# cvg/diffmvs

Measured on AMD Instinct MI355X. Metric: depth-maps/sec (640x512, 5 src views), higher is better.
Workload: dtype f32

## Files before the change

### diffmvs_amd/_lib.py

```python
from __future__ import annotations

import ctypes as C
import os

PKG = os.path.dirname(os.path.abspath(__file__))
HIP_LIB_PATH = os.environ.get("DMVS_LIB") or os.path.join(PKG, "libdmvs_hip.so")

ACT_NONE, ACT_RELU, ACT_SIGMOID, ACT_TANH, ACT_SILU = range(5)
IN_PLAIN, IN_UPSAMPLE2, IN_UNSHUFFLE2, IN_ZEROINSERT2 = range(4)
LAYOUT_NCHW, LAYOUT_NHWC, LAYOUT_NHWC_BF16, LAYOUT_NHWC_F16 = 0, 1, 2, 3
DTYPE_F32, DTYPE_BF16, DTYPE_F16, DTYPE_F32_PLAIN = 0, 1, 2, 3
ARITH_F32, ARITH_BF16, ARITH_SPLIT = 0, 1, 2
EW_DEPTH_TO_DISP, EW_DISP_TO_DEPTH = 0, 1

_P = C.c_void_p
_I = C.c_int32
_F = C.c_float


class Conv2dDesc(C.Structure):
    _fields_ = [
        ("in0", _P), ("in1", _P), ("mul0", _P), ("weight", _P), ("scale", _P), ("shift", _P),
        ("residual", _P), ("gru_z", _P), ("gru_h", _P), ("out", _P), ("gn_stats", _P), ("out_mul", _P),
        ("B", _I), ("c0", _I), ("c1", _I), ("Hin", _I), ("Win", _I), ("Hout", _I), ("Wout", _I),
# ... 13 lines not shown
    ]


class GetCostDesc(C.Structure):
    _fields_ = [
        ("ref", _P), ("src", _P), ("rt", _P), ("inv_depth", _P), ("confidence", _P), ("view_w", _P),
        ("disp_min", _P), ("disp_max", _P), ("out_cost", _P), ("out_samples", _P), ("worklist", _P),
        ("B", _I), ("S", _I), ("C", _I), ("G", _I), ("n", _I), ("H", _I), ("W", _I), ("vw_shift", _I),
        ("cost_cstride", _I), ("cost_coffset", _I), ("samp_cstride", _I), ("samp_coffset", _I),
        ("interval", _F), ("min_radius", _F), ("max_radius", _F), ("feat_dtype", _I), ("tune", _I),
    ]


SIGNATURES = {
    "dmvs_abi_version": [],
    "dmvs_conv2d_f32": [C.POINTER(Conv2dDesc), _P],
    "dmvs_featurenet_stem_f32": [_P, _P, _P, _P, _P, _P, _P, _P, _I, _I, _I, _I, _P],
    "dmvs_featurenet_stem3_f32": [_P, _P, _P, _P, _P, _P, _P, _P, _P, _P, _P, _I, _I, _I, _I, _P],
    "dmvs_featurenet_conv1_pair_f32": [_P, _P, _P, _P, _P, _P, _P, _P, _I, _I, _I, _I, _P],
    "dmvs_featurenet_fpn_tail_f32": [_P, _P, _P, _P, _P, _P, _I, _I, _I, _I, _P],
    "dmvs_conv2d_wgrad_workspace_f32": [C.POINTER(Conv2dDesc), C.POINTER(C.c_int64)],
    "dmvs_conv2d_wgrad_f32": [C.POINTER(Conv2dDesc), _P, _P, _P, _P, C.c_int64, _P],
    "dmvs_conv3d_f32": [C.POINTER(Conv3dDesc), _P],
    "dmvs_conv3d_wgrad_workspace_f32": [C.POINTER(Conv3dDesc), C.POINTER(C.c_int64)],
    "dmvs_conv3d_wgrad_f32": [C.POINTER(Conv3dDesc), _P, _P, _P, _P, C.c_int64, _P],
    "dmvs_compose_proj_f32": [_P, _P, _I, _I, _P],
    "dmvs_warp_volume_f32": [_P, _P, _P, _P, _I, _I, _I, _I, _I, _I, _I, _P],
    "dmvs_getcost_quad_f32": [C.POINTER(GetCostDesc), _P],
    "dmvs_warp_corr_init_quad_f32": [_P, _P, _P, _P, _P, _P, _I, _I, _I, _I, _I, _I, _I, _I, _I, _I, _I, _P],
    "dmvs_warp_corr_init_bwd_f32": [_P, _P, _P, _P, _P, _P, _P, _P, _I, _I, _I, _I, _I, _I, _I, _I, _I, _I, _P],
    "dmvs_getcost_bwd_f32": [C.POINTER(GetCostDesc), _P, _P, _P, _P],
    "dmvs_view_aggregate_bwd_f32": [_P, _P, _P, _P, _P, _P, _I, _I, _I, _I, _P],
    "dmvs_view_aggregate_f32": [_P, _P, _P, _I, _I, _I, _I, _P],
    "dmvs_sigmoid_max_d_f32": [_P, _P, _I, _I, _I, _P],
    "dmvs_depth_regress_f32": [_P, _P, _P, _P, _P, _P, _I, _I, _I, _P],
    "dmvs_convex_upsample_f32": [_P, _P, _P, _P, _P, _P, _I, _I, _I, _I, _P],
    "dmvs_mask_upsample4_f32": [_P, _P, _P, _F, _P, _P, _P, _P, _P, _I, _I, _I, _I, _I, _P],
    "dmvs_groupnorm_silu_f32": [_P, _P, _P, _P, _P, _P, _P, _I, _I, _I, _I, _F, _P],
    "dmvs_groupnorm_apply_f32": [_P, _P, _P, _P, _P, _P, _P, _I, _I, _I, _I, _F, _P],
    "dmvs_delta_update_f32": [_P, _P, _P, _F, _P, _P, _P, _I, _I, _I, _I, _P],
    "dmvs_depth_convert_f32": [_P, _P, _P, _P, _I, _I, _I, _P],
    "dmvs_act_slice_f32": [_P, _P, _I, _I, _I, _I, _I, _I, _I, _I, _P],
    "dmvs_upsample_nearest_f32": [_P, _P, _I, _I, _I, _I, _P],
    "dmvs_nchw_to_nhwc_f32": [_P, _P, _I, _I, _I, _P],
    "dmvs_groupnorm_silu_bwd_workspace_f32": [_I, _I, _I, C.POINTER(C.c_int64)],
    "dmvs_groupnorm_silu_bwd_f32": [_P, _P, _P, _P, _P, _P, _P, _P, _P, _P, _P, C.c_int64, _I, _I, _I, _I, _F, _P],
    "dmvs_batchnorm_workspace_f32": [_I, _I, _I, _I, C.POINTER(C.c_int64)],
    "dmvs_batchnorm_train_fwd_f32": [_P, _P, _P, _P, _P, _P, _P, _P, _P, C.c_int64, _I, _I, _I, _I, _I, _F, _F, _I, _P],
    "dmvs_batchnorm_train_bwd_f32": [_P, _P, _P, _P, _P, _P, _P, _P, _P, _P, C.c_int64, _I, _I, _I, _I, _I, _I, _P],
    "dmvs_geo_consistency_f32": [_P, _P, _P, _P, _P, _I, _I, _F, _F, _P, _P, _I, _I, _I, _I, _I, _P],
    "dmvs_sumsq_f32": [_P, C.c_int64, _P, _P],
    "dmvs_adamw_step_f32": [_P, _P, _P, _P, C.c_int64, _F, _F, _F, _F, _F, _I, _F, _P, _F, _P],
    "dmvs_view_select_scores_f64": [_P, _P, _P, _P, _P, C.c_int64, C.c_int64, _P, _I, C.c_double, C.c_double, C.c_double, _P, _P, _P],
    "dmvs_cloud_nn_dist_f32": [_P, C.c_int64, _P, C.c_int64, _P, _P, C.c_int64, _P, C.c_double, _P, _F, _P, _P, _P],
    "dmvs_cloud_stats_f32": [_P, _P, C.c_int64, _F, _P, _I, C.c_double, _I, _P, _P],
    "dmvs_cloud_nn_index_f32": [_P, C.c_int64, _P, C.c_int64, _P, _P, C.c_int64, _P, C.c_double, _P, _F, _P, _P, _P, _P, _P],
    "dmvs_cloud_pair_moments_f64": [_P, C.c_int64, _P, _P, C.c_int64, _P, _P, _F, _P, _P, C.c_double, C.c_double, C.c_double, _I, _P, _P],
    "dmvs_cloud_crop_prism_f32": [_P, C.c_int64, _P, _P, _I, _I, C.c_double, C.c_double, _P, _P],
    "dmvs_depth_stats_f32": [_P, _P, _P, C.c_int64, C.c_int64, _P, _I, C.c_double, C.c_double, C.c_double, C.c_double, _I, _P, _P],
    "dmvs_cloud_splat_zmin_f32": [_P, C.c_int64, _P, _P, C.c_int64, _I, _I, C.c_double, C.c_double, C.c_double, _I, _I, _P, _P, _P, _P],
    "dmvs_cloud_splat_sum_f32": [_P, C.c_int64, _P, _P, C.c_int64, _I, _I, C.c_double, C.c_double, C.c_double, C.c_double, C.c_double, _I, _P, _P, _P, _P],
    "dmvs_depth_normals_f32": [_P, _P, _P, C.c_int64, _I, _I, _I, C.c_double, _I, _P, _P, _P],
    "dmvs_tsdf_integrate_f32": [_P, _P, _P, _P, C.c_int64, _I, _I, _I, _I, _I, _P, C.c_double, C.c_double, _I, _P, _P, _P, _P],
    "dmvs_tsdf_flags_u8": [_P, _P, _I, _I, _I, _I, _P, _P, _P],
    "dmvs_tsdf_vertices_f32": [_P, _P, _P, _I, _I, _I, _P, C.c_double, _P, _P, C.c_int64, _P, _P, _P],
    "dmvs_tsdf_faces_i32": [_P, _I, _I, _I, _P, _P, _P, C.c_int64, _P, _P],
    "dmvs_mesh_raster_fill_u64": [_P, C.c_int64, _P],
    "dmvs_mesh_raster_zid_u64": [_P, C.c_int64, _P, C.c_int64, _P, _P, C.c_int64, _I, _I, _I, _I, _P, _P, _P, _P, C.c_int64, _P],
    "dmvs_mesh_raster_resolve_f32": [_P, _P, C.c_int64, _P, C.c_int64, _P, _P, C.c_int64, _I, _I, _P, _P, _P, _P, _P, _P],
    "dmvs_mesh_label_round_i32": [_P, C.c_int64, C.c_int64, _P, _P, _I, _P],
    "dmvs_mesh_face_tally_i64": [_P, C.c_int64, _P, C.c_int64, _P, C.c_double, C.c_double, _P, _P, _P, _I, _P],
    "dmvs_mesh_sample_f32": [_P, C.c_int64, _P, C.c_int64, _P, C.c_int64, C.c_int64, _P, _P, _I, _P],
}
VIEW_SELECT_MAX_IMAGES, VIEW_SELECT_MAX_LIST = 16384, 1 << 23
CLOUD_MAX_RINGS, CLOUD_MAX_KEY_BITS, CLOUD_MAX_THRESHOLDS = 1024, 62, 16
CLOUD_MOMENTS, CLOUD_MAX_POLYGON = 20, 256
DEPTH_MAX_THRESHOLDS, DEPTH_SLOTS = 8, 7
SPLAT_VIEW_CHUNK, SPLAT_VIEW_DOUBLES, SPLAT_SLOTS, SPLAT_MAX_RADIUS, SPLAT_NO_PRETEST = 8, 15, 4, 16, 0x1
NORMAL_MAX_RADIUS, NORMAL_CAM_DOUBLES, NORMAL_VIEW_CHUNK, NORMAL_SLOTS = 4, 27, 8, 4
TSDF_VIEW_CHUNK, TSDF_VIEW_DOUBLES, TSDF_MAX_VIEWS, TSDF_MAX_QUADS, TSDF_NO_CULL = 8, 12, 65535, 357913941, 0x1
RASTER_VIEW_DOUBLES, RASTER_SLOTS, RASTER_SMALL, RASTER_CULL_NEG, RASTER_CULL_POS = 22, 8, 64, 0x1, 0x2
ABI_VERSION = 4
TUNE_NO_WALK, TUNE_PIECES4, TUNE_NO_LEAN, TUNE_1X1_TILED, TUNE_NO_TALL, TUNE_TALL = 0x4, 0x8, 0x100, 0x200, 0x400, 0x800
TUNE3D_PIECES4, TUNE3D_S2_DIRECT, TUNE3D_NO_PAIR = 0x1, 0x2, 0x4
TUNE_SWEEP_GLOBAL = 0x1
TUNE_WGRAD_ACCUMULATE = 0x1000
TUNE_SPLIT_ALL = 0x20000
TUNE_STEM_EXACT = 0x40000


def tune_xcd_group(n: int) -> int:
    return (int(n) & 7) << 14


def tune3d_xcd_group(n: int) -> int:
    return (int(n) & 7) << 4
TUNE_BWD_INTERLEAVED, BWD_GATHER_INTERLEAVED = 0x1, 2


def tune_tile_wx(n: int) -> int:
    return n & 3


def tune_tile_mt(n: int) -> int:
    return (n & 7) << 4


class DmvsError(RuntimeError):
    pass


class Lib:

    def __init__(self, path: str):
        if not os.path.exists(path):
            raise DmvsError(f"{path} not found: build it with `python -m diffmvs_amd.build`")
        self.path = path
        self.dll = C.CDLL(path)
        self.dll.dmvs_abi_version.restype = C.c_int
        v = self.dll.dmvs_abi_version()
        if v != ABI_VERSION:
            raise DmvsError(f"{path}: ABI version {v}, binding expects {ABI_VERSION} (rebuild: python -m diffmvs_amd.build)")
        for name, argtypes in SIGNATURES.items():
            fn = getattr(self.dll, name)
            fn.argtypes = argtypes
            fn.restype = C.c_int

    def call(self, name: str, *args):
        rc = getattr(self.dll, name)(*args)
        if rc != 0:
            raise DmvsError(f"{name} failed with code {rc}" + (" (DMVS_EINVAL: unsupported descriptor)" if rc == -22 else " (hipError_t)"))


_hip_lib = None


def hip_lib() -> Lib:
    global _hip_lib
    if _hip_lib is None:
        _hip_lib = Lib(HIP_LIB_PATH)
    return _hip_lib
```

### diffmvs_amd/csrc/conv3d.hip

```cpp

#include <type_traits>

#include "dmvs_common.h"
#include "dmvs_lds_poison.h"

typedef float f32x4 __attribute__((ext_vector_type(4)));
typedef float f32x2 __attribute__((ext_vector_type(2)));

__device__ __forceinline__ int conv3d_xcd_tile(int tile, int ntiles, int tune) {
    const int xg = (tune >> 4) & 7;
    if (xg == 1) return tile;
    const unsigned g = xg == 0 ? 4u : (xg <= 4 ? 1u << (xg - 1) : 4u);
    return (int)dmvs_xcd_grouped_block((unsigned)tile, (unsigned)ntiles, g);
}

constexpr int pad16mod32_3d(int n) {
    int m = n;
    while (m % 32 != 16) ++m;
    return m;
}

constexpr unsigned kHaloGuard = 0x00808080u;

template <int ID, int IH, int IW, int PLANE_>
// ... 667 lines not shown
                __builtin_amdgcn_global_load_lds(srcp, DMVS_LDS_PTR(dstp), 16, 0, 0);
            }
        }
    };

    const int xr = tid / XT, lx = (tid - xr * XT) * 4;
    const int rd = xr / YT, ry = xr - rd * YT;
    const bool active = rd < DT;
    const int lbase = 4 + ((2 * rd) * IH + 2 * ry) * PW + lx;
    float acc[2][2][4];
#pragma unroll
    for (int i = 0; i < 16; ++i) (&acc[0][0][0])[i] = 0.0f;
    stage(0, lds);
    int cur = 0;
    for (int ci = 0; ci < d.cin; ++ci, cur ^= 1) {
        const float* s_in = lds + cur * plane + lbase;
        DMVS_DMA_BARRIER();
        if (ci + 1 < d.cin) stage(ci + 1, lds + (cur ^ 1) * plane);
        if (!active) continue;
        typedef const __attribute__((address_space(4))) float* cfloat_p;
        cfloat_p wc = (cfloat_p)(uintptr_t)(d.weight + ci * 27 * d.cout_pad);
        float w[27];
#pragma unroll
        for (int t = 0; t < 27; ++t) w[t] = wc[t * d.cout_pad];
#pragma unroll
        for (int dz = 0; dz < 4; ++dz) {
#pragma unroll
            for (int yy = 0; yy < 4; ++yy) {
                const float* row = s_in + (dz * IH + yy) * PW;
                const f32x4 mid = *reinterpret_cast<const f32x4*>(row);
                const float in6[6] = {row[-1], mid[0], mid[1], mid[2], mid[3], row[4]};
#pragma unroll
                for (int od = 0; od < 2; ++od) {
#pragma unroll
                    for (int oy = 0; oy < 2; ++oy) {
                        const int kd = dz - od, ky = yy - oy;
                        if (kd < 0 || kd > 2 || ky < 0 || ky > 2) continue;
                        const float w0 = w[(kd * 3 + ky) * 3], w1 = w[(kd * 3 + ky) * 3 + 1], w2 = w[(kd * 3 + ky) * 3 + 2];
#pragma unroll
                        for (int j = 0; j < 4; ++j)
                            acc[od][oy][j] = fmaf(in6[j], w0, fmaf(in6[j + 1], w1, fmaf(in6[j + 2], w2, acc[od][oy][j])));
                    }
                }
            }
        }
    }
    if (!active) return;
    const int ovol = d.Dout * d.Hout * d.Wout;
    const float sc = d.scale ? d.scale[0] : 1.0f, sh = d.shift ? d.shift[0] : 0.0f;
    float* outb = d.out + (size_t)b * ovol;
    const float* resb = d.residual ? d.residual + (size_t)b * ovol : nullptr;
#pragma unroll
    for (int od = 0; od < 2; ++od) {
#pragma unroll
        for (int oy = 0; oy < 2; ++oy) {
            const int gd = d0 + 2 * rd + od, gy = y0 + 2 * ry + oy;
            if (gd >= d.Dout || gy >= d.Hout) continue;
            const int o0 = (gd * d.Hout + gy) * d.Wout + lx;
            f32x4 y;
#pragma unroll
            for (int j = 0; j < 4; ++j) y[j] = dmvs_act(acc[od][oy][j] * sc + sh, d.act);
            if (resb) y += *reinterpret_cast<const f32x4*>(resb + o0);
            *reinterpret_cast<f32x4*>(outb + o0) = y;
        }
    }
}

static bool c1_rows_shape(const dmvs_conv3d_desc& d, int& XT, int& YT, int& DT) {
    if (d.Win % 4 || d.Win < 16 || d.Win > 256) return false;
    if (((uintptr_t)d.in | (uintptr_t)d.out | (uintptr_t)d.residual) & 15) return false;
    XT = d.Win / 4;
    const int RT = DMVS_BLOCK / XT;
    long best_tiles = -1, best_rows = 0;
    for (int yt = 1; yt <= 4 && yt <= RT; ++yt)
        for (int dt = 1; dt <= 4 && yt * dt <= RT; ++dt) {
            const long rows = (long)(2 * yt + 2) * (2 * dt + 2);
            if (2 * (rows * (d.Win + 4) + 4) > kC1RowsLds || rows * (XT + 1) + 1 > kC1RowsPieces * DMVS_BLOCK) continue;
            const long tiles = (long)((d.Hout + 2 * yt - 1) / (2 * yt)) * ((d.Dout + 2 * dt - 1) / (2 * dt));
            if (best_tiles < 0 || tiles < best_tiles || (tiles == best_tiles && tiles * rows < best_rows)) {
                best_tiles = tiles; best_rows = tiles * rows; YT = yt; DT = dt;
            }
        }
    return best_tiles > 0;
}


template <int CO>
__device__ __forceinline__ void conv3d_epilogue(const dmvs_conv3d_desc& d, const float (&acc)[CO], int co0, int b,
                                                size_t ovox) {
    const size_t ovol = (size_t)d.Dout * d.Hout * d.Wout;
#pragma unroll
    for (int co = 0; co < CO; ++co) {
        const int cg = co0 + co;
        if (cg >= d.cout) break;
        float y = acc[co];
        if (d.scale) y *= d.scale[cg];
        if (d.shift) y += d.shift[cg];
        y = dmvs_act(y, d.act);
        const size_t oi = ((size_t)b * d.cout + cg) * ovol + ovox;
        if (d.residual) y += d.residual[oi];
        d.out[oi] = y;
    }
}

template <int CO, int STRIDE>
__global__ void __launch_bounds__(DMVS_BLOCK) conv3d_kernel(const dmvs_conv3d_desc d) {
    const long total = (long)d.B * d.Dout * d.Hout * d.Wout;
    const long p = (long)blockIdx.x * DMVS_BLOCK + threadIdx.x;
    const int co0 = blockIdx.y * CO;
    const bool live = p < total;
    long q = live ? p : total - 1;
    const int ox = (int)(q % d.Wout); q /= d.Wout;
    const int oy = (int)(q % d.Hout); q /= d.Hout;
    const int od = (int)(q % d.Dout);
    const int b = (int)(q / d.Dout);

    float acc[CO];
#pragma unroll
    for (int i = 0; i < CO; ++i) acc[i] = 0.0f;
    const size_t ivol = (size_t)d.Din * d.Hin * d.Win;
    const int id0 = od * STRIDE - 1, iy0 = oy * STRIDE - 1, ix0 = ox * STRIDE - 1;
    for (int ci = 0; ci < d.cin; ++ci) {
        const float* vol = d.in + ((size_t)b * d.cin + ci) * ivol;
        const float* wrow = d.weight + (size_t)ci * 27 * d.cout_pad + co0;
#pragma unroll
        for (int kd = 0; kd < 3; ++kd) {
            const int id = id0 + kd;
            const bool din = id >= 0 && id < d.Din;
#pragma unroll
            for (int ky = 0; ky < 3; ++ky) {
                const int iy = iy0 + ky;
                const bool yin = din && iy >= 0 && iy < d.Hin;
#pragma unroll
                for (int kx = 0; kx < 3; ++kx) {
                    const int ix = ix0 + kx;
                    float v = 0.0f;
                    if (yin && ix >= 0 && ix < d.Win) v = vol[((size_t)id * d.Hin + iy) * d.Win + ix];
                    const float* wt = wrow + ((kd * 3 + ky) * 3 + kx) * d.cout_pad;
#pragma unroll
                    for (int co = 0; co < CO; ++co) acc[co] = fmaf(v, wt[co], acc[co]);
                }
            }
        }
    }
    if (!live) return;
    conv3d_epilogue<CO>(d, acc, co0, b, ((size_t)od * d.Hout + oy) * d.Wout + ox);
}

template <int CO>
__global__ void __launch_bounds__(DMVS_BLOCK) deconv3d_kernel(const dmvs_conv3d_desc d) {
    const long total = (long)d.B * d.Din * d.Hin * d.Win;
    const long p = (long)blockIdx.x * DMVS_BLOCK + threadIdx.x;
    const int co0 = blockIdx.y * CO;
    const int pd = (blockIdx.z >> 2) & 1, py = (blockIdx.z >> 1) & 1, px = blockIdx.z & 1;
    const bool live = p < total;
    long q = live ? p : total - 1;
    const int jx = (int)(q % d.Win); q /= d.Win;
    const int jy = (int)(q % d.Hin); q /= d.Hin;
    const int jd = (int)(q % d.Din);
    const int b = (int)(q / d.Din);

    float acc[CO];
#pragma unroll
    for (int i = 0; i < CO; ++i) acc[i] = 0.0f;
    const size_t ivol = (size_t)d.Din * d.Hin * d.Win;
    const int nd = pd ? 2 : 1, ny = py ? 2 : 1, nx = px ? 2 : 1;
// ... 107 lines not shown
    const int jx = jx0 + m, jd = jd0 + wave;
    const bool live = jx < d.Win && jd < d.Din;
    float* outb = d.out + (size_t)b * d.cout * ovol;
    const float* resb = d.residual ? d.residual + (size_t)b * d.cout * ovol : nullptr;
#pragma unroll
    for (int r = 0; r < 4; ++r) {
        const int cg = cg0 + r;
        const bool okc = cg < d.cout;
        const float sc = d.scale ? d.scale[okc ? cg : 0] : 1.0f, sh = d.shift ? d.shift[okc ? cg : 0] : 0.0f;
#pragma unroll
        for (int c2 = 0; c2 < 2; ++c2) {
#pragma unroll
            for (int mt = 0; mt < 4; ++mt) {
                const float keep = lowhalf ? acc[c2][mt][r] : acc[c2 + 2][mt][r];
                const float give = lowhalf ? acc[c2 + 2][mt][r] : acc[c2][mt][r];
                const float got = __shfl_xor(give, 32, 64);
                const int c = lowhalf ? c2 : c2 + 2;
                const int jy = jy0 + mt;
                if (!live || !okc || jy >= d.Hin) continue;
                const int o = cg * ovol + ((2 * jd + (c >> 1)) * d.Hout + 2 * jy + (c & 1)) * d.Wout + 2 * jx;
                float v0 = dmvs_act((lowhalf ? keep : got) * sc + sh, d.act);
                float v1 = dmvs_act((lowhalf ? got : keep) * sc + sh, d.act);
                if (resb) {
                    const float2 rv = *reinterpret_cast<const float2*>(resb + o);
                    v0 += rv.x;
                    v1 += rv.y;
                }
                *reinterpret_cast<float2*>(outb + o) = make_float2(v0, v1);
            }
        }
    }
}

static bool conv3d_s2_mfma(const dmvs_conv3d_desc& d) { return !(d.tune & DMVS_TUNE3D_S2_DIRECT); }

extern "C" int dmvs_conv3d_f32(const dmvs_conv3d_desc* dp, void* stream) {
    if (!dp) return DMVS_EINVAL;
    const dmvs_conv3d_desc& d = *dp;
    hipStream_t st = (hipStream_t)stream;
    if (d.cout_pad % 8 || d.cout > d.cout_pad || !d.in || !d.weight || !d.out) return DMVS_EINVAL;
    if ((uintptr_t)d.weight & 15) return DMVS_EINVAL;
    const int co = (d.cout_pad % 16 == 0) ? 16 : 8;
    dim3 block(DMVS_BLOCK);
    if (d.transposed) {
        if (d.stride != 2 || d.Dout != 2 * d.Din || d.Hout != 2 * d.Hin || d.Wout != 2 * d.Win) return DMVS_EINVAL;
        const long total = (long)d.B * d.Din * d.Hin * d.Win;
        if ((long)d.cout * d.Dout * d.Hout * d.Wout < (1L << 31) && (long)d.cin * d.Din * d.Hin * d.Win < (1L << 31)) {
            const int tiles_x = (d.Win + 15) / 16, tiles_y = (d.Hin + 3) / 4, tiles_d = (d.Din + 3) / 4;
            dim3 g((unsigned)(tiles_x * tiles_y * tiles_d * d.B), (unsigned)((d.cout + 7) / 8));
            hipLaunchKernelGGL(deconv3d_mfma_kernel, g, block, 0, st, d, tiles_x, tiles_y, tiles_d);
            return dmvs_launch_status();
        }
        dim3 grid(dmvs_ceil_div(total, DMVS_BLOCK), d.cout_pad / co, 8);
        if (co == 16) hipLaunchKernelGGL((deconv3d_kernel<16>), grid, block, 0, st, d);
        else hipLaunchKernelGGL((deconv3d_kernel<8>), grid, block, 0, st, d);
        return dmvs_launch_status();
    }
    if (d.stride != 1 && d.stride != 2) return DMVS_EINVAL;
    const int ed = (d.Din - 1) / d.stride + 1, eh = (d.Hin - 1) / d.stride + 1, ew = (d.Win - 1) / d.stride + 1;
    if (ed != d.Dout || eh != d.Hout || ew != d.Wout) return DMVS_EINVAL;
    const long total = (long)d.B * d.Dout * d.Hout * d.Wout;
    dim3 grid(dmvs_ceil_div(total, DMVS_BLOCK), d.cout_pad / co);
    if (d.stride == 1 && ((long)d.cin * d.Din * d.Hin * d.Win >= (1L << 31) || (long)d.cout * d.Dout * d.Hout * d.Wout >= (1L << 31)))
        return DMVS_EINVAL;
    if (d.stride == 1 && d.cout == 1) {
        int XT, YT, DT;
        if (c1_rows_shape(d, XT, YT, DT)) {
            const int tiles_y = (d.Hout + 2 * YT - 1) / (2 * YT), tiles_d = (d.Dout + 2 * DT - 1) / (2 * DT);
            dim3 g((unsigned)(tiles_y * tiles_d * d.B));
            hipLaunchKernelGGL(conv3d_c1_rows_kernel, g, block, 0, st, d, XT, YT, DT, tiles_y, tiles_d);
            return dmvs_launch_status();
        }
        const int tiles_x = (d.Wout + 15) / 16, tiles_y = (d.Hout + 15) / 16, tiles_d = (d.Dout + 15) / 16;
        dim3 g((unsigned)(tiles_x * tiles_y * tiles_d * d.B));
        hipLaunchKernelGGL(conv3d_c1_kernel, g, block, 0, st, d, tiles_x, tiles_y, tiles_d);
        return dmvs_launch_status();
    }
    if (d.stride == 1) {
        const int tiles_x = (d.Wout + 15) / 16, tiles_y = (d.Hout + 3) / 4, tiles_d = (d.Dout + 3) / 4;
        const int ntiles = (d.cout_pad + 15) / 16;
        dim3 g((unsigned)(tiles_x * tiles_y * tiles_d * d.B), (unsigned)((ntiles + 1) / 2));
        const long vtiles = (long)tiles_x * tiles_y * tiles_d * d.B;
        const bool v16 = conv3d_v16_ok(d);
        if (!(d.tune & DMVS_TUNE3D_NO_PAIR) && d.cin <= 4 && d.cout <= 8 && d.cout_pad == 8) {
            const int tiles_d8 = (d.Dout + 7) / 8;
            if ((long)tiles_x * tiles_y * tiles_d8 * d.B >= 512) {
                if (v16) {
                    static const int resident = dmvs_resident_workgroups(reinterpret_cast<const void*>(conv3d_mfma_stream_pair_kernel<true>));
                    hipLaunchKernelGGL((conv3d_mfma_stream_pair_kernel<true>), dim3((unsigned)resident, 1), block, 0, st, d, tiles_x, tiles_y, tiles_d8);
                } else {
                    hipLaunchKernelGGL((conv3d_mfma_stream_pair_kernel<false>), dim3((unsigned)(256 * kPairWgsPerCu), 1), block, 0, st, d, tiles_x, tiles_y, tiles_d8);
                }
                return dmvs_launch_status();
            }
        }
        if (!(d.tune & DMVS_TUNE3D_NO_PAIR) && v16 && d.cin > 4 && d.cin <= 8 && d.cout <= 8 && d.cout_pad == 8) {
            const int tiles_d8 = (d.Dout + 7) / 8;
            if ((long)tiles_x * tiles_y * tiles_d8 * d.B >= 512) {
                static const int resident = dmvs_resident_workgroups(reinterpret_cast<const void*>(conv3d_mfma_stream_pair8_kernel));
                hipLaunchKernelGGL(conv3d_mfma_stream_pair8_kernel, dim3((unsigned)resident, 1), block, 0, st, d, tiles_x, tiles_y, tiles_d8);
                return dmvs_launch_status();
            }
        }
        if (d.cin <= 4 && ntiles == 1 && vtiles >= 256 * kStreamWgsPerCu) {
            dim3 gs((unsigned)(256 * kStreamWgsPerCu), 1);
            if (v16) hipLaunchKernelGGL((conv3d_mfma_stream_kernel<1, true>), dim3(256 * 4, 1), block, 0, st, d, tiles_x, tiles_y, tiles_d);
            else hipLaunchKernelGGL((conv3d_mfma_stream_kernel<1>), gs, block, 0, st, d, tiles_x, tiles_y, tiles_d);
            return dmvs_launch_status();
        }
        if (v16) {
            if (ntiles == 1) hipLaunchKernelGGL((conv3d_mfma_kernel<1, 1, true>), g, block, 0, st, d, tiles_x, tiles_y, tiles_d);
            else hipLaunchKernelGGL((conv3d_mfma_kernel<2, 1, true>), g, block, 0, st, d, tiles_x, tiles_y, tiles_d);
        } else if (ntiles == 1) hipLaunchKernelGGL((conv3d_mfma_kernel<1>), g, block, 0, st, d, tiles_x, tiles_y, tiles_d);
        else hipLaunchKernelGGL((conv3d_mfma_kernel<2>), g, block, 0, st, d, tiles_x, tiles_y, tiles_d);
    } else {
        const bool fits32 = (long)d.cin * d.Din * d.Hin * d.Win < (1L << 31) && (long)d.cout * d.Dout * d.Hout * d.Wout < (1L << 31);
        const int ntiles = (d.cout_pad + 15) / 16;
        if (fits32 && ntiles <= 2 && conv3d_s2_mfma(d)) {
            const int tiles_x = (d.Wout + 15) / 16, tiles_y = (d.Hout + 3) / 4, tiles_d = (d.Dout + 3) / 4;
            dim3 g((unsigned)(tiles_x * tiles_y * tiles_d * d.B), 1);
            if (ntiles == 1) hipLaunchKernelGGL((conv3d_mfma_kernel<1, 2>), g, block, 0, st, d, tiles_x, tiles_y, tiles_d);
            else hipLaunchKernelGGL((conv3d_mfma_kernel<2, 2>), g, block, 0, st, d, tiles_x, tiles_y, tiles_d);
            return dmvs_launch_status();
        }
        if (co == 16) hipLaunchKernelGGL((conv3d_kernel<16, 2>), grid, block, 0, st, d);
        else hipLaunchKernelGGL((conv3d_kernel<8, 2>), grid, block, 0, st, d);
    }
    return dmvs_launch_status();
}

template <int S>
__global__ void __launch_bounds__(DMVS_BLOCK) conv3d_wgrad_kernel(const dmvs_conv3d_desc d, const float* __restrict__ gout,
                                                                  float* __restrict__ ws, int want_bias, int tiles_x, int tiles_y,
                                                                  int tiles_d) {
    constexpr int CK = S == 1 ? 8 : 2;
    constexpr int IW = 15 * S + 3, IH = 3 * S + 3, ID = 3 * S + 3;
    constexpr int PLANE = pad16mod32_3d(ID * IH * IW);
    constexpr int GROW = 257;
    constexpr int NTN = (CK * 27 + 1 + 15) / 16;
    constexpr int IN_IT = (CK * PLANE + DMVS_BLOCK - 1) / DMVS_BLOCK, G_IT = (16 * GROW + DMVS_BLOCK - 1) / DMVS_BLOCK;
    __shared__ float lds[CK * PLANE + 16 * GROW];
    DMVS_LDS_POISON(lds);
    float* s_in = lds;
    float* s_g = lds + CK * PLANE;
    const int tid = threadIdx.x, lane = tid & 63, wave = tid >> 6;
    const int m = lane & 15, kq = lane >> 4;
    const int c0 = blockIdx.y * CK, cobase = blockIdx.z * 16;
    const size_t ivol = (size_t)d.Din * d.Hin * d.Win, ovol = (size_t)d.Dout * d.Hout * d.Wout;
    const int vol = (int)ivol;
    int boff[NTN];
#pragma unroll
    for (int nt = 0; nt < NTN; ++nt) {
        const int jj = nt * 16 + m;
        const int ci = jj / 27, t = jj - ci * 27;
        boff[nt] = jj < CK * 27 ? ci * PLANE + ((t / 9) * IH + (t / 3) % 3) * IW + t % 3 : 0;
    }
    f32x4 acc[NTN];
#pragma unroll
    for (int nt = 0; nt < NTN; ++nt) acc[nt] = f32x4{0.0f, 0.0f, 0.0f, 0.0f};
    const float bias_one = (want_bias && blockIdx.y == 0) ? 1.0f : 0.0f;
    const int ntiles = tiles_x * tiles_y * tiles_d * d.B;
    for (int tile = blockIdx.x; tile < ntiles; tile += gridDim.x) {
        int tq = tile;
        const int tx = tq % tiles_x; tq /= tiles_x;
        const int ty = tq % tiles_y; tq /= tiles_y;
        const int td = tq % tiles_d;
// ... 152 lines not shown
```

### diffmvs_amd/ops.py

```python
from __future__ import annotations

import ctypes as C
import os
from dataclasses import dataclass
from typing import Optional

import torch

from . import _lib
from ._lib import (ACT_NONE, ACT_RELU, ACT_SIGMOID, ACT_SILU, ACT_TANH, ARITH_BF16, ARITH_F32, ARITH_SPLIT, DTYPE_BF16, DTYPE_F16, DTYPE_F32, IN_PLAIN,
                   IN_UNSHUFFLE2, IN_UPSAMPLE2, IN_ZEROINSERT2, LAYOUT_NCHW, LAYOUT_NHWC, LAYOUT_NHWC_BF16, LAYOUT_NHWC_F16)

CONV_ARITH = {"fp32": ARITH_F32, "bf16": ARITH_BF16, "split": ARITH_SPLIT}
FEATURE_DTYPES = {"fp32": torch.float32, "bf16": torch.bfloat16, "fp16": torch.float16}
_DTYPE_CODE = {torch.float32: DTYPE_F32, torch.bfloat16: DTYPE_BF16, torch.float16: DTYPE_F16}
_NHWC_LAYOUT = {torch.float32: LAYOUT_NHWC, torch.bfloat16: LAYOUT_NHWC_BF16, torch.float16: LAYOUT_NHWC_F16}


def _round_up(x: int, m: int) -> int:
    return (x + m - 1) // m * m


@dataclass
class PackedConv:
# ... 46 lines not shown
    cout, cin, kh, kw = w.shape
    cp = _pad_cout(cout)
    if cp == cout:
        wk = w.permute(1, 2, 3, 0).contiguous()
    else:
        wk = torch.zeros(cin, kh, kw, cp, dtype=torch.float32, device=w.device)
        wk[..., :cout] = w.permute(1, 2, 3, 0)
    scale = shift = None
    if bn is not None:
        scale, shift = fold_bn(bn)
        if bias is not None:
            shift = shift + bias.detach().float() * scale
    elif bias is not None:
        shift = bias.detach().float()
    pad = (pad, pad) if isinstance(pad, int) else tuple(pad)
    return PackedConv(wk.contiguous(), None if scale is None else scale.contiguous().float(),
                      None if shift is None else shift.contiguous().float(), cin, cout, cp, (kh, kw), stride, pad)


def pack_conv3d(w: torch.Tensor, bias=None, bn: Optional[dict] = None, stride=1, transposed=False) -> PackedConv:
    w = w.detach().float()
    if transposed:
        cin, cout = w.shape[0], w.shape[1]
        wk_src = w.permute(0, 2, 3, 4, 1)
    else:
        cout, cin = w.shape[0], w.shape[1]
        wk_src = w.permute(1, 2, 3, 4, 0)
    cp = _pad_cout(cout)
    if cp == cout:
        wk = wk_src.reshape(cin, 27, cout).contiguous()
    else:
        wk = torch.zeros(cin, 27, cp, dtype=torch.float32, device=w.device)
        wk[..., :cout] = wk_src.reshape(cin, 27, cout)
    scale = shift = None
    if bn is not None:
        scale, shift = fold_bn(bn)
    elif bias is not None:
        shift = bias.detach().float()
    return PackedConv(wk.contiguous(), None if scale is None else scale.contiguous(),
                      None if shift is None else shift.contiguous(), cin, cout, cp, (3, 3, 3), stride, (1, 1),
                      transposed)


def g4_channels(C: int, dtype=torch.float32) -> torch.Tensor:
    p = torch.arange(C)
    if dtype != torch.float32:
        return p
    return ((p // 4) % 4) * (C // 4) + (p // 16) * 4 + p % 4


def _ptr(t: Optional[torch.Tensor]):
    return None if t is None else C.c_void_p(t.data_ptr())


MAX_WINDOW_VIEWS = 16
RASTER_QUEUE_ENTRIES = 1 << 20

_weights_generation = [0]


def weights_generation() -> int:
    return _weights_generation[0]


def bump_weights_generation() -> None:
    _weights_generation[0] += 1


BWD_INTERLEAVED_DEFAULT = 1


def _env_tune():
    e = os.environ.get
    t2 = _lib.tune_tile_wx(int(e("DMVS_CONV_WX", "0"))) | _lib.tune_tile_mt(int(e("DMVS_CONV_MT", "0")))
    t2 |= _lib.TUNE_NO_WALK if e("DMVS_CONV_WALK") == "0" else 0
    t2 |= _lib.TUNE_PIECES4 if e("DMVS_CONV_V16") == "0" else 0
    t2 |= _lib.TUNE_NO_LEAN if e("DMVS_CONV_LEAN") == "0" else 0
    t2 |= _lib.TUNE_1X1_TILED if e("DMVS_CONV1X1_PX4") == "0" else 0
    t2 |= {"0": _lib.TUNE_NO_TALL, "1": _lib.TUNE_TALL}.get(e("DMVS_CONV_TALL"), 0)
    t2 |= _lib.TUNE_SPLIT_ALL if e("DMVS_CONV_SPLIT_ALL") == "1" else 0
    t2 |= _lib.tune_xcd_group(int(e("DMVS_CONV_XCD", "0")))
    t3 = (_lib.TUNE3D_PIECES4 if e("DMVS_CONV3D_V16") == "0" else 0) | (_lib.TUNE3D_S2_DIRECT if e("DMVS_CONV3D_S2") == "direct" else 0)
    t3 |= _lib.TUNE3D_NO_PAIR if e("DMVS_CONV3D_PAIR") == "0" else 0
    t3 |= _lib.tune3d_xcd_group(int(e("DMVS_CONV3D_XCD", "0")))
    return {"conv2d": t2, "conv3d": t3, "stem": (_lib.TUNE_PIECES4 if e("DMVS_STEM_V16") == "0" else 0) | _lib.tune_xcd_group(int(e("DMVS_STEM_XCD", "0"))) | (_lib.TUNE_STEM_EXACT if e("DMVS_STEM_EXACT") == "1" else 0),
            "sweep": _lib.TUNE_SWEEP_GLOBAL if e("DMVS_PLANE_SWEEP") == "quad" else 0,
            "bwd_gather": e("DMVS_GETCOST_BWD") == "gather",
            "bwd_il": e("DMVS_BWD_INTERLEAVED", "%d" % BWD_INTERLEAVED_DEFAULT) == "1"}


class Ops:
    _bindings = {}

    def __init__(self, lib: _lib.Lib, device):
        self.lib = lib
        self.device = torch.device(device)
        self.tune = _env_tune()
        self.timers = None
        self.conv_arith = ARITH_F32
        self.debug_fill = None
        self.getcost_hook = None

    def with_conv_arith(self, arith: int) -> "Ops":
        import copy
        o = copy.copy(self)
        o.conv_arith = arith
        return o

    def _call(self, name, *args):
        if self.timers is not None and name in self.timers:
            st, en = torch.cuda.Event(enable_timing=True), torch.cuda.Event(enable_timing=True)
            st.record()
            self.lib.call(name, *args)
            en.record()
            self.timers[name].append((st, en))
        else:
            self.lib.call(name, *args)

    @classmethod
    def for_device(cls, device) -> "Ops":
        device = torch.device(device)
        if device.type != "cuda":
            raise _lib.DmvsError(
                f"diffmvs_amd runs on MI355X only (got device '{device}'); there is no CPU path. "
                "Move the model and inputs to a HIP device.")
        if device.index is None:
            device = torch.device("cuda", torch.cuda.current_device())
        lib = _lib.hip_lib()
        key = (lib.path, device.index)
        o = cls._bindings.get(key)
        if o is None:
            o = cls._bindings[key] = cls(lib, device)
        return o

    def stream(self):
        if self.device.type == "cuda":
            return C.c_void_p(torch.cuda.current_stream(self.device).cuda_stream)
        return None

    def empty(self, *shape, dtype=torch.float32):
        t = torch.empty(*shape, dtype=dtype, device=self.device)
        if self.debug_fill is not None and t.is_floating_point():
            t.fill_(self.debug_fill)
        return t

    def empty_like(self, x):
        t = torch.empty_like(x)
        if self.debug_fill is not None and t.is_floating_point():
            t.fill_(self.debug_fill)
        return t

    def _chk_feat(self, *ts):
        dt = ts[0].dtype
        for t in ts:
            if t.dtype not in _DTYPE_CODE or t.dtype != dt or not t.is_contiguous() or t.device != self.device:
                raise _lib.DmvsError(f"expected contiguous fp32 / bf16 / fp16 feature tensors of one dtype on {self.device}, got "
                                     f"{t.dtype} contiguous={t.is_contiguous()} on {t.device}")
        return _DTYPE_CODE[dt]

    def _chk(self, *ts):
        for t in ts:
            if t is None:
                continue
            if t.dtype != torch.float32 or not t.is_contiguous() or t.device != self.device:
                raise _lib.DmvsError(f"expected contiguous fp32 tensor on {self.device}, got {t.dtype} "
                                     f"contiguous={t.is_contiguous()} on {t.device}")
# ... 857 lines not shown
```

### include/dmvs.h

```cpp
#ifndef DMVS_H
#define DMVS_H

#include <stdint.h>

#ifdef __cplusplus
extern "C" {
#endif

#define DMVS_ABI_VERSION 4
#define DMVS_EINVAL (-22)

enum { DMVS_ACT_NONE = 0, DMVS_ACT_RELU = 1, DMVS_ACT_SIGMOID = 2, DMVS_ACT_TANH = 3, DMVS_ACT_SILU = 4 };
enum { DMVS_IN_PLAIN = 0, DMVS_IN_UPSAMPLE2 = 1 , DMVS_IN_UNSHUFFLE2 = 2 ,
       DMVS_IN_ZEROINSERT2 = 3  };
enum { DMVS_LAYOUT_NCHW = 0, DMVS_LAYOUT_NHWC = 1,
       DMVS_LAYOUT_NHWC_BF16 = 2, DMVS_LAYOUT_NHWC_F16 = 3 };
enum { DMVS_DTYPE_F32 = 0 , DMVS_DTYPE_BF16 = 1, DMVS_DTYPE_F16 = 2 ,
       DMVS_DTYPE_F32_PLAIN = 3  };

int dmvs_abi_version(void);

#define DMVS_ARITH_F32 0
#define DMVS_ARITH_BF16 1
#define DMVS_ARITH_SPLIT 2
// ... 1 lines not shown
#define DMVS_TUNE_TILE_WX(n) ((n) & 3)
#define DMVS_TUNE_NO_WALK 0x4
#define DMVS_TUNE_PIECES4 0x8
#define DMVS_TUNE_TILE_MT(n) (((n) & 7) << 4)
#define DMVS_TUNE_1X1_TILED 0x200
#define DMVS_TUNE_NO_LEAN 0x100
#define DMVS_TUNE_TALL(n) (((n) & 3) << 10)
#define DMVS_TUNE_STEM_EXACT 0x40000
#define DMVS_TUNE_SPLIT_ALL 0x20000
#define DMVS_TUNE_XCD_GROUP(n) (((n) & 7) << 14)

typedef struct dmvs_conv2d_desc {
    const float* in0;
    const float* in1;
    const float* mul0;
    const float* weight;
    const float* scale;
    const float* shift;
    const float* residual;
    const float* gru_z;
    const float* gru_h;
    float* out;
    double* gn_stats;
    const float* out_mul;
    int32_t B, c0, c1;
    int32_t Hin, Win;
    int32_t Hout, Wout;
    int32_t cout, cout_pad;
    int32_t kh, kw, stride, pad_h, pad_w;
    int32_t in_mode, act;
    int32_t res_mode;
    int32_t res_after_act;
    int32_t out_layout, out_cstride, out_coffset;
    int32_t gn_groups;
    float post_scale;
    int32_t gate_cstride;
    int32_t arith;
    int32_t tune;
    int32_t out_mul_c0;
    int32_t in0_cstride;
    const void* weight_split;
} dmvs_conv2d_desc;

int dmvs_conv2d_f32(const dmvs_conv2d_desc* d, void* stream);

int dmvs_featurenet_stem_f32(const float* x, const float* w0, const float* scale0, const float* shift0, const float* w1,
                             const float* scale1, const float* shift1, float* y, int32_t N, int32_t H, int32_t W, int32_t tune,
                             void* stream);

int dmvs_featurenet_stem3_f32(const float* x, const float* w0, const float* scale0, const float* shift0, const float* w1,
                              const float* scale1, const float* shift1, const float* w2, const float* scale2, const float* shift2,
                              float* y, int32_t N, int32_t H, int32_t W, int32_t tune, void* stream);

int dmvs_featurenet_conv1_pair_f32(const float* x, const void* wsplit1, const float* scale1, const float* shift1, const void* wsplit2,
                                   const float* scale2, const float* shift2, float* y, int32_t N, int32_t H, int32_t W, int32_t tune,
                                   void* stream);

int dmvs_featurenet_fpn_tail_f32(const float* c2, const float* c3, const float* w_inner, const float* b_inner, const void* wsplit_out,
                                 float* y, int32_t N, int32_t H, int32_t W, int32_t tune, void* stream);

#define DMVS_TUNE_WGRAD_ACCUMULATE 0x1000
int dmvs_conv2d_wgrad_workspace_f32(const dmvs_conv2d_desc* d, int64_t* bytes);
int dmvs_conv2d_wgrad_f32(const dmvs_conv2d_desc* d, const float* grad_out, float* gw, float* gb, float* workspace,
                          int64_t workspace_bytes, void* stream);

typedef struct dmvs_conv3d_desc {
    const float* in;
    const float* weight;
    const float* scale;
    const float* shift;
    const float* residual;
    float* out;
    int32_t B, cin, cout, cout_pad;
    int32_t Din, Hin, Win;
    int32_t Dout, Hout, Wout;
    int32_t stride;
    int32_t transposed;
    int32_t act;
    int32_t tune;
} dmvs_conv3d_desc;
#define DMVS_TUNE3D_PIECES4 0x1
#define DMVS_TUNE3D_S2_DIRECT 0x2
#define DMVS_TUNE3D_NO_PAIR 0x4
#define DMVS_TUNE3D_XCD_GROUP(n) (((n) & 7) << 4)

int dmvs_conv3d_f32(const dmvs_conv3d_desc* d, void* stream);

int dmvs_conv3d_wgrad_workspace_f32(const dmvs_conv3d_desc* d, int64_t* bytes);
int dmvs_conv3d_wgrad_f32(const dmvs_conv3d_desc* d, const float* grad_out, float* gw, float* gb, float* workspace,
                          int64_t workspace_bytes, void* stream);

int dmvs_compose_proj_f32(const float* proj, float* out, int32_t B, int32_t V, void* stream);

#define DMVS_GETCOST_TILE 16
#define DMVS_GETCOST_MAX_WINDOW_VIEWS 16
#define DMVS_GETCOST_WORKLIST_INTS(B, H, W) \
    (4 + 66 * (B) * (((H) + DMVS_GETCOST_TILE - 1) / DMVS_GETCOST_TILE) * (((W) + DMVS_GETCOST_TILE - 1) / DMVS_GETCOST_TILE))
typedef struct dmvs_getcost_desc {
    const float* ref;
    const float* src;
    const float* rt;
    const float* inv_depth;
    const float* confidence;
    const float* view_w;
    const float* disp_min;
    const float* disp_max;
    float* out_cost;
    float* out_samples;
    int32_t* worklist;
    int32_t B, S, C, G, n, H, W;
    int32_t vw_shift;
    int32_t cost_cstride, cost_coffset, samp_cstride, samp_coffset;
    float interval, min_radius, max_radius;
    int32_t feat_dtype;
    int32_t tune;
} dmvs_getcost_desc;

#define DMVS_TUNE_SWEEP_GLOBAL 0x1
int dmvs_getcost_quad_f32(const dmvs_getcost_desc* d, void* stream);
int dmvs_warp_corr_init_quad_f32(const void* ref, const void* src, const float* rt,
                                 const float* disp_min, const float* disp_max, float* out,
                                 int32_t B, int32_t S, int32_t C, int32_t G, int32_t D,
                                 int32_t H, int32_t W, int32_t Hs, int32_t Ws, int32_t feat_dtype, int32_t tune, void* stream);

int dmvs_warp_volume_f32(const float* src, const float* rt, const float* depth, float* out,
                         int32_t B, int32_t C, int32_t D, int32_t H, int32_t W, int32_t Hs, int32_t Ws,
                         void* stream);

#define DMVS_TUNE_BWD_INTERLEAVED 0x1
#define DMVS_BWD_GATHER_INTERLEAVED 2
int dmvs_warp_corr_init_bwd_f32(const float* ref, const float* src, const float* rt,
                                const float* disp_min, const float* disp_max, const float* gcor,
                                float* gref, float* gsrc, int32_t B, int32_t S, int32_t C, int32_t G,
                                int32_t D, int32_t H, int32_t W, int32_t Hs, int32_t Ws, int32_t gather, void* stream);
int dmvs_getcost_bwd_f32(const dmvs_getcost_desc* d, const float* gcost, float* gref, float* gsrc, void* stream);
int dmvs_view_aggregate_bwd_f32(const float* cor, const float* w, const float* out, const float* gout,
                                float* gcor, float* gw, int32_t B, int32_t S, int32_t GD, int32_t HW,
                                void* stream);

int dmvs_view_aggregate_f32(const float* cor, const float* w, float* out,
                            int32_t B, int32_t S, int32_t GD, int32_t HW, void* stream);

int dmvs_sigmoid_max_d_f32(const float* x, float* out, int32_t N, int32_t D, int32_t HW, void* stream);

int dmvs_depth_regress_f32(const float* logits, const float* disp_min, const float* disp_max,
                           float* norm_depth, float* depth, float* conf,
                           int32_t B, int32_t D, int32_t HW, void* stream);

int dmvs_convex_upsample_f32(const float* inv, const float* mask, const float* disp_min,
                             const float* disp_max, float* out_inv, float* out_depth,
                             int32_t B, int32_t H, int32_t W, int32_t ratio, void* stream);

int dmvs_mask_upsample4_f32(const float* x, const float* weight, const float* bias, float post_scale, const float* inv,
                            const float* disp_min, const float* disp_max, float* out_inv, float* out_depth,
                            int32_t B, int32_t cin, int32_t cout_pad, int32_t H, int32_t W, void* stream);

int dmvs_groupnorm_silu_f32(const float* x, const float* gamma, const float* beta,
                            const float* scale_shift, const float* residual, float* y,
                            double* stats, int32_t B, int32_t C, int32_t HW, int32_t groups,
                            float eps, void* stream);

int dmvs_groupnorm_apply_f32(const float* x, const float* gamma, const float* beta,
                             const float* scale_shift, const float* residual, float* y,
                             const double* stats, int32_t B, int32_t C, int32_t HW, int32_t groups,
                             float eps, void* stream);

// ... 132 lines not shown
```

Baseline: 1562.

## Add persistent depth-marching VALU kernel for small-cin 8-output 3D convs

Adds a persistent 3D conv kernel for stride-1 convs with cin<=4 and cout_pad 8. Each workgroup marches along depth over a height band, keeping a four-slot ring of input depth slices in LDS that is filled by async global-to-LDS loads. Each slice is loaded once and reused across the three kd taps, and the FMAs use packed f32x2 VALU instead of the MFMA pair kernel. The output store is deferred one step so it overlaps the next compute step. It takes priority over the existing MFMA pair path by default and can be disabled with an env flag, at the cost of running on vector ALUs instead of matrix cores.

```diff
diff --git a/diffmvs_amd/_lib.py b/diffmvs_amd/_lib.py
--- a/diffmvs_amd/_lib.py
+++ b/diffmvs_amd/_lib.py
@@ -119,7 +119,7 @@
 RASTER_VIEW_DOUBLES, RASTER_SLOTS, RASTER_SMALL, RASTER_CULL_NEG, RASTER_CULL_POS = 22, 8, 64, 0x1, 0x2
 ABI_VERSION = 4
 TUNE_NO_WALK, TUNE_PIECES4, TUNE_NO_LEAN, TUNE_1X1_TILED, TUNE_NO_TALL, TUNE_TALL = 0x4, 0x8, 0x100, 0x200, 0x400, 0x800
-TUNE3D_PIECES4, TUNE3D_S2_DIRECT, TUNE3D_NO_PAIR = 0x1, 0x2, 0x4
+TUNE3D_PIECES4, TUNE3D_S2_DIRECT, TUNE3D_NO_PAIR, TUNE3D_NO_VALU8 = 0x1, 0x2, 0x4, 0x8
 TUNE_SWEEP_GLOBAL = 0x1
 TUNE_WGRAD_ACCUMULATE = 0x1000
 TUNE_SPLIT_ALL = 0x20000
diff --git a/diffmvs_amd/csrc/conv3d.hip b/diffmvs_amd/csrc/conv3d.hip
--- a/diffmvs_amd/csrc/conv3d.hip
+++ b/diffmvs_amd/csrc/conv3d.hip
@@ -773,6 +773,208 @@
             }
         }
     return best_tiles > 0;
+}
+
+constexpr int kMarchLds = 19200;
+constexpr int kMarchPieces = 5;
+constexpr int kMarchMaxBand = 16;
+constexpr int kMarchMinChunk = 12;
+constexpr long kMarchUnitsPerWg = 16;
+
+struct MarchShape {
+    int XT, BH, DC, nbands, ndc;
+};
+struct MarchUnit {
+    int b, y0, d0, nin;
+};
+__device__ __forceinline__ MarchUnit march_unit(int u, const MarchShape& s, int D) {
+    MarchUnit m;
+    const int band = u % s.nbands;
+    u /= s.nbands;
+    const int dc = u % s.ndc;
+    m.b = u / s.ndc;
+    m.y0 = band * s.BH;
+    m.d0 = dc * s.DC;
+    m.nin = min(s.DC, D - m.d0) + 2;
+    return m;
+}
+
+__device__ __forceinline__ void march_fma2(f32x2& acc, float in, f32x2 w) {
+#ifdef DMVS_HOST_EMULATION
+    acc[0] = fmaf(in, w[0], acc[0]);
+    acc[1] = fmaf(in, w[1], acc[1]);
+#else
+    acc = __builtin_elementwise_fma(f32x2{in, in}, w, acc);
+#endif
+}
+
+template <int CIN>
+__global__ void __launch_bounds__(DMVS_BLOCK) conv3d_c8_march_kernel(const dmvs_conv3d_desc d, const MarchShape s) {
+    __shared__ __attribute__((aligned(16))) float lds[kMarchLds];
+    DMVS_LDS_POISON(lds);
+    const int tid = threadIdx.x, wave = __builtin_amdgcn_readfirstlane(tid >> 6);
+    const int W = d.Win, H = d.Hin, D = d.Din, hw = H * W, vol = D * hw;
+    const int PW = W + 4, NP = s.XT + 1;
+    const int plane = (s.BH + 2) * PW + 4, slice = CIN * plane;
+    const int npc = plane / 4, npieces = CIN * npc;
+    const int nunits = d.B * s.nbands * s.ndc;
+
+    int pcol[kMarchPieces], prow[kMarchPieces];
+    int off[kMarchPieces];
+#pragma unroll
+    for (int it = 0; it < kMarchPieces; ++it) {
+        const int pe = it * DMVS_BLOCK + tid;
+        const int c = pe / npc, q = pe - c * npc - 1;
+        const int row = q / NP, xi = q - row * NP;
+        pcol[it] = pe >= npieces ? -2 : (q >= 0 && xi < s.XT) ? c * vol + 4 * xi : -1;
+        prow[it] = row;
+    }
+    MarchUnit lu = {0, 0, 0, 0}, cu = {0, 0, 0, 0};
+    int lnext = blockIdx.x, lj = 0;
+    auto load_unit = [&]() {
+        lu = march_unit(lnext, s, D);
+        lnext += gridDim.x;
+        lj = 0;
+#pragma unroll
+        for (int it = 0; it < kMarchPieces; ++it) {
+            const int gy = lu.y0 - 1 + prow[it];
+            off[it] = pcol[it] < 0 ? pcol[it] : (gy >= 0 && gy < H) ? pcol[it] + gy * W : -1;
+        }
+    };
+    bool ldone = lnext >= nunits;
+    auto stage_next = [&](int slot) {
+        const int gd = lu.d0 - 1 + lj;
+        const bool din = gd >= 0 && gd < D;
+        const float* base = d.in + (size_t)lu.b * CIN * vol + (din ? gd * hw : 0);
+        float* buf = lds + slot * slice;
+#pragma unroll
+        for (int it = 0; it < kMarchPieces; ++it) {
+            if (off[it] != -2) {
+                const float* srcp = (din && off[it] >= 0) ? base + off[it] : dmvs_zero16;
+                float* dstp = buf + (it * DMVS_BLOCK + wave * 64) * 4;
+                __builtin_amdgcn_global_load_lds(srcp, DMVS_LDS_PTR(dstp), 16, 0, 0);
+            }
+        }
+        if (++lj == lu.nin) {
+            if (lnext < nunits) load_unit();
+            else ldone = true;
+        }
+    };
+
+    const int xr = tid / s.XT, lx = (tid - xr * s.XT) * 4;
+    const int lbase = 4 + xr * PW + lx;
+    const int ovol = d.Dout * d.Hout * d.Wout;
+    float sc[8], sh[8];
+#pragma unroll
+    for (int co = 0; co < 8; ++co) {
+        sc[co] = d.scale ? d.scale[co < d.cout ? co : 0] : 1.0f;
+        sh[co] = d.shift ? d.shift[co < d.cout ? co : 0] : 0.0f;
+    }
+    typedef const __attribute__((address_space(4))) float* cfloat_p;
+    cfloat_p wc = (cfloat_p)(uintptr_t)d.weight;
+
+    f32x2 pend[4][4];
+    size_t pend_o = 0;
+    bool have = false, pact = false;
+    auto store = [&]() {
+#pragma unroll
+        for (int co = 0; co < 8; ++co) {
+            if (co >= d.cout) break;
+            const size_t o = pend_o + (size_t)co * ovol;
+            f32x4 y;
+#pragma unroll
+            for (int r = 0; r < 4; ++r) y[r] = pend[co >> 1][r][co & 1] * sc[co] + sh[co];
+            if (d.act == DMVS_ACT_RELU) {
+#pragma unroll
+                for (int r = 0; r < 4; ++r) y[r] = fmaxf(y[r], 0.0f);
+            } else if (d.act != DMVS_ACT_NONE) {
+#pragma unroll
+                for (int r = 0; r < 4; ++r) y[r] = dmvs_act(y[r], d.act);
+            }
+            if (d.residual) y += *reinterpret_cast<const f32x4*>(d.residual + o);
+            *reinterpret_cast<f32x4*>(d.out + o) = y;
+        }
+    };
+
+    if (ldone) return;
+    ldone = false;
+    load_unit();
+    cu = lu;
+    int cnext = blockIdx.x + gridDim.x, cj = 0;
+    stage_next(0);
+    for (int q = 0;; ++q) {
+        DMVS_DMA_BARRIER();
+        if (!ldone) stage_next((q + 1) & 3);
+        if (have && pact) store();
+        have = false;
+        if (cj >= 2) {
+            const int od = cu.d0 + cj - 2, oy = cu.y0 + xr;
+            pact = xr < s.BH && oy < H;
+            have = true;
+            pend_o = (size_t)cu.b * d.cout * ovol + (size_t)((od * H + oy) * W + lx);
+            if (pact) {
+                f32x2 acc[4][4];
+#pragma unroll
+                for (int i = 0; i < 16; ++i) (&acc[0][0])[i] = f32x2{0.0f, 0.0f};
+#pragma unroll 1
+                for (int kd = 0; kd < 3; ++kd) {
+                    const float* sp = lds + ((q + 2 + kd) & 3) * slice + lbase;
+                    cfloat_p wk = wc + kd * 72;
+#pragma unroll
+                    for (int ky = 0; ky < 3; ++ky) {
+                        float in6[CIN][6];
+#pragma unroll
+                        for (int ci = 0; ci < CIN; ++ci) {
+                            const float* row = sp + ci * plane + ky * PW;
+                            const f32x4 mid = *reinterpret_cast<const f32x4*>(row);
+                            in6[ci][0] = row[-1]; in6[ci][1] = mid[0]; in6[ci][2] = mid[1]; in6[ci][3] = mid[2]; in6[ci][4] = mid[3]; in6[ci][5] = row[4];
+                        }
+#pragma unroll
+                        for (int kx = 0; kx < 3; ++kx) {
+#pragma unroll
+                            for (int ci = 0; ci < CIN; ++ci) {
+                                f32x2 w2[4];
+#pragma unroll
+                                for (int cp = 0; cp < 4; ++cp) {
+                                    w2[cp][0] = wk[(ci * 27 + ky * 3 + kx) * 8 + 2 * cp];
+                                    w2[cp][1] = wk[(ci * 27 + ky * 3 + kx) * 8 + 2 * cp + 1];
+                                }
+#pragma unroll
+                                for (int j = 0; j < 4; ++j)
+#pragma unroll
+                                    for (int cp = 0; cp < 4; ++cp) march_fma2(acc[cp][j], in6[ci][j + kx], w2[cp]);
+                            }
+                        }
+                    }
+                }
+#pragma unroll
+                for (int i = 0; i < 16; ++i) (&pend[0][0])[i] = (&acc[0][0])[i];
+            }
+        }
+        if (++cj == cu.nin) {
+            if (cnext >= nunits) break;
+            cu = march_unit(cnext, s, D);
+            cnext += gridDim.x;
+            cj = 0;
+        }
+    }
+    if (have && pact) store();
+}
+
+static bool c8_march_shape(const dmvs_conv3d_desc& d, int resident, MarchShape& s) {
+    if (d.tune & (DMVS_TUNE3D_NO_PAIR | DMVS_TUNE3D_NO_VALU8)) return false;
+    if (d.cin < 1 || d.cin > 4 || d.cout > 8 || d.cout_pad != 8) return false;
+    if (d.Win % 4 || d.Win < 16 || d.Win > 256) return false;
+    if (((uintptr_t)d.in | (uintptr_t)d.out | (uintptr_t)d.residual) & 15) return false;
+    s.XT = d.Win / 4;
+    const int lds_rows = (kMarchLds / (4 * d.cin) - 4) / (d.Win + 4) - 2;
+    s.BH = std::min(std::min(DMVS_BLOCK / s.XT, kMarchMaxBand), std::min(lds_rows, (int)d.Hin));
+    if (s.BH < 1) return false;
+    s.nbands = (d.Hin + s.BH - 1) / s.BH;
+    s.DC = d.Din;
+    while (s.DC > kMarchMinChunk && (long)d.B * s.nbands * ((d.Din + s.DC - 1) / s.DC) < kMarchUnitsPerWg * resident) s.DC = (s.DC + 1) / 2;
+    s.ndc = (d.Din + s.DC - 1) / s.DC;
+    return true;
 }
 
 
@@ -1046,6 +1248,21 @@
         dim3 g((unsigned)(tiles_x * tiles_y * tiles_d * d.B), (unsigned)((ntiles + 1) / 2));
         const long vtiles = (long)tiles_x * tiles_y * tiles_d * d.B;
         const bool v16 = conv3d_v16_ok(d);
+        {
+            static const int resident = dmvs_resident_workgroups(reinterpret_cast<const void*>(conv3d_c8_march_kernel<4>));
+            MarchShape ms;
+            if (c8_march_shape(d, resident, ms)) {
+                const long units = (long)d.B * ms.nbands * ms.ndc;
+                const dim3 gm((unsigned)std::min<long>(units, resident), 1);
+                switch (d.cin) {
+                    case 1: hipLaunchKernelGGL((conv3d_c8_march_kernel<1>), gm, block, 0, st, d, ms); break;
+                    case 2: hipLaunchKernelGGL((conv3d_c8_march_kernel<2>), gm, block, 0, st, d, ms); break;
+                    case 3: hipLaunchKernelGGL((conv3d_c8_march_kernel<3>), gm, block, 0, st, d, ms); break;
+                    default: hipLaunchKernelGGL((conv3d_c8_march_kernel<4>), gm, block, 0, st, d, ms); break;
+                }
+                return dmvs_launch_status();
+            }
+        }
         if (!(d.tune & DMVS_TUNE3D_NO_PAIR) && d.cin <= 4 && d.cout <= 8 && d.cout_pad == 8) {
             const int tiles_d8 = (d.Dout + 7) / 8;
             if ((long)tiles_x * tiles_y * tiles_d8 * d.B >= 512) {
diff --git a/diffmvs_amd/ops.py b/diffmvs_amd/ops.py
--- a/diffmvs_amd/ops.py
+++ b/diffmvs_amd/ops.py
@@ -152,6 +152,7 @@
     t2 |= _lib.tune_xcd_group(int(e("DMVS_CONV_XCD", "0")))
     t3 = (_lib.TUNE3D_PIECES4 if e("DMVS_CONV3D_V16") == "0" else 0) | (_lib.TUNE3D_S2_DIRECT if e("DMVS_CONV3D_S2") == "direct" else 0)
     t3 |= _lib.TUNE3D_NO_PAIR if e("DMVS_CONV3D_PAIR") == "0" else 0
+    t3 |= _lib.TUNE3D_NO_VALU8 if e("DMVS_CONV3D_VALU8") == "0" else 0
     t3 |= _lib.tune3d_xcd_group(int(e("DMVS_CONV3D_XCD", "0")))
     return {"conv2d": t2, "conv3d": t3, "stem": (_lib.TUNE_PIECES4 if e("DMVS_STEM_V16") == "0" else 0) | _lib.tune_xcd_group(int(e("DMVS_STEM_XCD", "0"))) | (_lib.TUNE_STEM_EXACT if e("DMVS_STEM_EXACT") == "1" else 0),
             "sweep": _lib.TUNE_SWEEP_GLOBAL if e("DMVS_PLANE_SWEEP") == "quad" else 0,
diff --git a/include/dmvs.h b/include/dmvs.h
--- a/include/dmvs.h
+++ b/include/dmvs.h
@@ -107,6 +107,7 @@
 #define DMVS_TUNE3D_PIECES4 0x1
 #define DMVS_TUNE3D_S2_DIRECT 0x2
 #define DMVS_TUNE3D_NO_PAIR 0x4
+#define DMVS_TUNE3D_NO_VALU8 0x8
 #define DMVS_TUNE3D_XCD_GROUP(n) (((n) & 7) << 4)
 
 int dmvs_conv3d_f32(const dmvs_conv3d_desc* d, void* stream);
```

Result: no change. 1562 (-0.0%).
